# jameshensman/pyvb

Measured on NVIDIA B200. Metric: VB-PCA missing-data rows*iters/sec, higher is better.
Workload: dtype f64

## Files before the change

### pyvb_b200/csrc/kernels_i8.cu

```cuda
#include <cuda.h>
#include <stdio.h>
#include <stdlib.h>

#include "common.cuh"
#include "kernels.h"
#include "ptx.cuh"
#include "umma.cuh"

namespace pyvb {

namespace {

__host__ __device__ constexpr int i_tri(int i) { return i * (i + 1) / 2; }
__host__ __device__ constexpr int i_nc8(int q) { return (i_tri(q) + 31) & ~31; }
constexpr int NPL = 7;
constexpr int BM = 128, BKB = 64, ST = 16, CT = 32;
constexpr int A_B = BM * BKB, B_B = NPL * CT * BKB;
constexpr int NTHR = 10 * 32;

__device__ __forceinline__ double pow2_above(double m) {
    if (!(m > 0.0 && m < 1e300)) return 1.0;
    int e;
    frexp(m, &e);
    return ldexp(1.0, e);
// ... 657 lines not shown
            hi[k] = (unsigned int)(u >> 32);
        }
#pragma unroll
        for (int p = 0; p < NPL; ++p) {
            const unsigned int *w = (p < 4) ? lo : hi;
            const unsigned int sel = (unsigned)(p & 3) | ((unsigned)(4 + (p & 3)) << 4);
            const unsigned int w01 = __byte_perm(w[0], w[1], sel), w23 = __byte_perm(w[2], w[3], sel);
            *reinterpret_cast<unsigned int *>(&sh[(p * CT + lane) * PITCH + r]) = __byte_perm(w01, w23, 0x5410);
        }
    }
    __syncthreads();
    const int nct = gridDim.y;
#pragma unroll
    for (int h = 0; h < 2; ++h) {
        const long long kb = n0 / 64 + h;
        unsigned int *dst = reinterpret_cast<unsigned int *>(ZI + ((size_t)(kb * nct + ct) * (NPL * CT)) * 64);
        for (int w = threadIdx.x; w < NPL * CT * 16; w += 256)
            dst[w] = *reinterpret_cast<const unsigned int *>(&sh[(w >> 4) * PITCH + h * 64 + (w & 15) * 4]);
    }
}

__global__ void __launch_bounds__(256)
prepare_maskT_kernel(long long N, int D, long long npad, const double *__restrict__ X, long long ldx,
                     signed char *__restrict__ maskT) {
    constexpr int PITCH = 132;
    __shared__ __align__(16) signed char sh[32 * PITCH];
    const int d0 = blockIdx.y * 32;
    const long long n0 = (long long)blockIdx.x * 128;
    const int lane = threadIdx.x & 31, warp = threadIdx.x >> 5;
    const int d = d0 + lane;
    for (int r = warp; r < 128; r += 8) {
        const long long n = n0 + r;
        signed char m = 0;
        if (d < D && n < N) {
            const double x = X[n * ldx + d];
            m = (x == x) ? 1 : 0;
        }
        sh[lane * PITCH + r] = m;
    }
    __syncthreads();
#pragma unroll
    for (int h = 0; h < 2; ++h) {
        const long long kb = n0 / 64 + h;
        for (int w = threadIdx.x; w < 32 * 16; w += 256) {
            const int row = w >> 4;
            if (d0 + row < D)
                *reinterpret_cast<unsigned int *>(maskT + ((size_t)kb * D + d0 + row) * 64 + (w & 15) * 4) =
                    *reinterpret_cast<const unsigned int *>(&sh[row * PITCH + h * 64 + (w & 15) * 4]);
        }
    }
}

constexpr int CHK_BLOCKS = 0;
__global__ void __launch_bounds__(128)
stats_i8_check_kernel(int D, int q, const double *__restrict__ ws, int nchunks, const double *__restrict__ cnt,
                      const double *__restrict__ zscale, double *__restrict__ guard, double tol) {
    __shared__ double sh[8];
    const StatLayout L(D, q);
    const int P = i_tri(q), warp = threadIdx.x >> 5, lane = threadIdx.x & 31;
    const int d = blockIdx.x;
    double sz = 0.0;
    for (int c = threadIdx.x; c < P; c += 128) sz = fmax(sz, zscale[c]);
    double dm = 0.0;
    for (int i = warp; i < q; i += 4) {
        const size_t off = L.t1 + (size_t)d * P + i_tri(i) + i;
        double t = 0.0;
        for (int ch = lane; ch < nchunks; ch += 32) t += ws[(size_t)ch * L.len + off];
        dm = fmax(dm, warp_sum(t));
    }
    for (int o = 16; o > 0; o >>= 1) sz = fmax(sz, __shfl_xor_sync(0xffffffffu, sz, o));
    if (lane == 0) {
        sh[warp] = sz;
        sh[4 + warp] = dm;
    }
    __syncthreads();
    if (threadIdx.x == 0) {
        sz = fmax(fmax(sh[0], sh[1]), fmax(sh[2], sh[3])) * 2.7755575615628914e-17;
        dm = fmax(fmax(sh[4], sh[5]), fmax(sh[6], sh[7]));
        if (cnt[d] * sz > tol * dm) atomicAdd(guard + 3, 1.0);
        __threadfence();
        const unsigned int done = atomicAdd(reinterpret_cast<unsigned int *>(guard + 2), 1u);
        if (done == gridDim.x - 1) {
            __threadfence();
            const double t = *reinterpret_cast<volatile double *>(guard + 3);
            guard[0] = t;
            if (t > 0.0) guard[1] += 1.0;
            guard[3] = 0.0;
            *reinterpret_cast<unsigned int *>(guard + 2) = 0u;
        }
    }
}

size_t si8_smem_bytes(int q, int pair = 0) {
    const int ns = pair ? SST_PAIR : SST;
    return 1024 + (size_t)ns * (A_B + (pair ? B_B / 2 : B_B)) + (size_t)((i_tri(q) + q + 31) & ~31) * 8 + (size_t)(2 * ns + 4) * 8 + 16;
}

template <int CL, bool PAIR = false>
__global__ void __launch_bounds__(NTHR, 1)
stats_i8_kernel(const __grid_constant__ CUtensorMap tmA, const __grid_constant__ CUtensorMap tmB, long long N, int D, int q,
                const double *__restrict__ zscale, double *__restrict__ ws, long long rows_per_chunk, int nchunks, int ndb,
                int nct, int ks) {
    extern __shared__ unsigned char smem_dyn[];
    unsigned char *smem = smem_dyn + ((1024u - (smem_u32(smem_dyn) & 1023u)) & 1023u);
    static_assert(!PAIR || CL == 2, "a CTA pair is a cluster of two");
    constexpr int BSZ = PAIR ? B_B / 2 : B_B, STG = A_B + BSZ, NSMAX = PAIR ? SST_PAIR : SST;
    const int NS = NSMAX / ks, SB = ks * STG;
    const int P = i_tri(q), NCZ = (P + q + 31) & ~31;
    unsigned char *st_base = smem;
    double *fcol = reinterpret_cast<double *>(smem + (size_t)NSMAX * STG);
    uint64_t *full = reinterpret_cast<uint64_t *>(fcol + NCZ);
    uint64_t *empty = full + NSMAX;
    uint64_t *tfull = empty + NSMAX;
    uint64_t *tempty = tfull + 2;
    uint32_t *tbase = reinterpret_cast<uint32_t *>(tempty + 2);

    const int tid = threadIdx.x, warp = tid >> 5, lane = tid & 31;
    const int crank = (CL > 1) ? (int)cluster_ctarank() : 0;
    const int ndg = (ndb + CL - 1) / CL;
    const int nitems = ndg * nct * nchunks;
    const int cid = (int)blockIdx.x / CL, ncl = (int)gridDim.x / CL;
    constexpr uint16_t CMASK = (uint16_t)((1u << CL) - 1u);
    for (int c = tid; c < NCZ; c += NTHR) fcol[c] = zscale[c] * 5.5511151231257827e-17;
    if (tid == 0) {
        tma_prefetch_desc(&tmA);
        tma_prefetch_desc(&tmB);
        for (int s = 0; s < NSMAX; ++s) {
            mbar_init(&full[s], 1);
            mbar_init(&empty[s], PAIR ? 1 : CL);
        }
        for (int b = 0; b < 2; ++b) {
            mbar_init(&tfull[b], 1);
            mbar_init(&tempty[b], PAIR ? 16 : 8);
        }
        mbar_fence_init();
    }
    if (warp == 1) {
        if (PAIR) umma::tmem_alloc2(tbase, 512);
        else umma::tmem_alloc(tbase, 512);
    }
    umma::fence_before_sync();
    __syncthreads();
    if (CL > 1) cluster_sync_all();
    umma::fence_after_sync();
    const uint32_t tmem = *tbase;

    auto item_geom = [&](int item, int &chunk, int &db, int &ct, long long &r0, int &nsteps) {
        chunk = item / (ndg * nct);
        const int rem = item - chunk * (ndg * nct);
        const int dg = rem / nct;
        ct = rem - dg * nct;
        db = dg * CL + crank;
        r0 = (long long)chunk * rows_per_chunk;
        long long r1 = r0 + rows_per_chunk;
        if (r1 > N) r1 = N;
        nsteps = (r1 > r0) ? (int)((r1 - r0 + BKB - 1) / BKB) : 0;
    };

    if (warp == 0) {
        const bool leader = elect_one();
        const uint32_t full_l = PAIR ? umma::map_to_cta(full, 0) : 0u;
        int s = 0;
        uint32_t ph = 0;
        for (int item = cid; item < nitems; item += ncl) {
            int chunk, db, ct, nsteps;
            long long r0;
            item_geom(item, chunk, db, ct, r0, nsteps);
            for (int k = 0; k < nsteps; k += ks) {
                const int kc = (nsteps - k < ks) ? nsteps - k : ks;
                umma::mbar_wait_bounded(&empty[s], ph ^ 1);
                if (leader) {
                    if (PAIR) {
                        if (crank == 0) mbar_arrive_expect_tx(&full[s], (uint32_t)(2 * kc * STG));
                    } else {
                        mbar_arrive_expect_tx(&full[s], (uint32_t)(kc * (A_B + B_B)));
                    }
                    for (int h = 0; h < kc; ++h) {
                        unsigned char *st = st_base + (size_t)s * SB + (size_t)h * STG;
                        const long long kb = r0 / BKB + k + h;
                        if (PAIR) {
                            tma_load_3d_i8_pair(st, &tmA, 0, (int)(kb * D + db * BM), 0, full_l + (uint32_t)s * 8u);
                            tma_load_3d_i8_pair(st + A_B, &tmB, 0, (int)((kb * nct + ct) * (NPL * CT) + crank * (NPL * CT / 2)), 0,
                                                full_l + (uint32_t)s * 8u);
                        } else {
                            tma_load_3d_i8(st, &tmA, 0, (int)(kb * D + db * BM), 0, &full[s]);
                            if (CL == 1)
                                tma_load_3d_i8(st + A_B, &tmB, 0, (int)((kb * nct + ct) * (NPL * CT)), 0, &full[s]);
                            else
                                tma_load_3d_i8_mc(st + A_B + crank * (B_B / CL), &tmB, 0,
                                                  (int)((kb * nct + ct) * (NPL * CT) + crank * (NPL * CT / CL)), 0, &full[s], CMASK);
                        }
                    }
                }
                __syncwarp();
                if (++s == NS) {
                    s = 0;
                    ph ^= 1;
                }
            }
        }
    } else if (warp == 1) {
        const bool leader = elect_one() && (!PAIR || crank == 0);
        const uint32_t idesc = umma::idesc_s8_s32(PAIR ? 2 * BM : BM, NPL * CT);
        const uint64_t adesc0 = umma::desc_kmajor_sw64(smem_u32(st_base), 0), bdesc0 = umma::desc_kmajor_sw64(smem_u32(st_base + A_B), 0);
        int s = 0, tl = 0;
        uint32_t ph = 0;
        for (int item = (PAIR && crank != 0) ? nitems : cid; item < nitems; item += ncl, ++tl) {
            int chunk, db, ct, nsteps;
            long long r0;
            item_geom(item, chunk, db, ct, r0, nsteps);
            const int buf = tl & 1;
            umma::mbar_wait_bounded(&tempty[buf], (uint32_t)(((tl >> 1) & 1) ^ 1));
            umma::fence_after_sync();
            const uint32_t dacc = tmem + (uint32_t)(buf * 256);
            for (int k = 0; k < nsteps; k += ks) {
                const int kc = (nsteps - k < ks) ? nsteps - k : ks;
                umma::mbar_wait_bounded(&full[s], ph);
                umma::fence_after_sync();
                if (leader) {
                    for (int h = 0; h < kc; ++h) {
                        const uint64_t off = (uint64_t)((s * SB + h * STG) >> 4);
                        if (PAIR) {
                            umma::mma_i8_pair(dacc, adesc0 + off, bdesc0 + off, idesc, (k + h) ? 1u : 0u);
                            umma::mma_i8_pair(dacc, adesc0 + off + 2, bdesc0 + off + 2, idesc, 1u);
                        } else {
                            umma::mma_i8(dacc, adesc0 + off, bdesc0 + off, idesc, (k + h) ? 1u : 0u);
                            umma::mma_i8(dacc, adesc0 + off + 2, bdesc0 + off + 2, idesc, 1u);
                        }
                    }
                    if (PAIR) umma::mma_commit_pair(&empty[s]);
                    else if (CL == 1) umma::mma_commit(&empty[s]);
                    else mma_commit_mc(&empty[s], CMASK);
                }
                __syncwarp();
                if (++s == NS) {
                    s = 0;
                    ph ^= 1;
                }
            }
            if (leader) {
                if (PAIR) umma::mma_commit_pair(&tfull[buf]);
                else umma::mma_commit(&tfull[buf]);
            }
            __syncwarp();
        }
    } else {
        const StatLayout L(D, q);
        const int wq = warp & 3, half = (warp - 2) >> 2;
        const uint32_t tempty_l = PAIR ? umma::map_to_cta(tempty, 0) : 0u;
        int tl = 0;
        for (int item = cid; item < nitems; item += ncl, ++tl) {
            int chunk, db, ct, nsteps;
            long long r0;
            item_geom(item, chunk, db, ct, r0, nsteps);
            const int buf = tl & 1;
            const int d = db * BM + wq * 32 + lane;
            const int c0 = ct * CT + half * 16;
            double *out = ws + (size_t)chunk * L.len;
            umma::mbar_wait_bounded(&tfull[buf], (uint32_t)((tl >> 1) & 1));
            umma::fence_after_sync();
            const uint32_t taddr = tmem + (uint32_t)(buf * 256 + half * 16) + ((uint32_t)(wq * 32) << 16);
#pragma unroll
            for (int ch = 0; ch < 2; ++ch) {
                uint32_t a[NPL][8];
                if (nsteps > 0) {
#pragma unroll
                    for (int p = 0; p < NPL; ++p) tmem_ld8(taddr + (uint32_t)(p * CT + ch * 8), a[p]);
                    umma::tmem_ld_wait();
                }
#pragma unroll
                for (int k = 0; k < 8; ++k) {
                    double v = 0.0;
                    if (nsteps > 0) {
#pragma unroll
                        for (int p = NPL - 1; p >= 0; --p) v = fma(v, 256.0, i2d((int)a[p][k]));
                    }
                    const int c = c0 + ch * 8 + k;
                    if (d < D) {
                        if (c < P) out[L.t1 + (size_t)d * P + c] = fcol[c] * v;
                        else if (c < P + q) out[L.bst + (size_t)d * q + (c - P)] = fcol[c] * v;
                    }
                }
            }
            umma::fence_before_sync();
            __syncwarp();
            if (lane == 0) {
                if (PAIR) umma::mbar_arrive_cluster(tempty_l + (uint32_t)buf * 8u);
                else mbar_arrive(&tempty[buf]);
            }
        }
    }
    umma::fence_before_sync();
    __syncthreads();
    if (CL > 1) cluster_sync_all();
    if (warp == 1) {
        if (PAIR) umma::tmem_dealloc2(tmem, 512);
        else umma::tmem_dealloc(tmem, 512);
    }
}

constexpr int SF_CONV = 8;
constexpr int SF_NTHR = (2 + 8 + SF_CONV) * 32;
constexpr int SF_STG = 2 * A_B + B_B;
constexpr int SF_NSMAX = 8;

int sf_stages(int q) {
    const size_t fixed = 1024 + (size_t)stats_i8_ncols(q) * 8 + (size_t)(2 * SF_NSMAX + 2) * 8 + 16;
    const int ns = (int)((227 * 1024 - fixed) / SF_STG);
    return ns < SF_NSMAX ? ns : SF_NSMAX;
}
size_t sf_smem_bytes(int q, int ns) {
    return 1024 + (size_t)ns * SF_STG + (size_t)stats_i8_ncols(q) * 8 + (size_t)(2 * ns + 2) * 8 + 16;
}

__global__ void __launch_bounds__(SF_NTHR, 1)
stats_i8_fused_kernel(const __grid_constant__ CUtensorMap tmA, long long N, int D, int q, const double *__restrict__ MZ, int ldmz,
                      const double *__restrict__ zscale, double *__restrict__ ws, long long rows_per_chunk, int nchunks,
                      int ndb, int nct, int ns) {
    extern __shared__ unsigned char smem_dyn[];
    unsigned char *smem = smem_dyn + ((1024u - (smem_u32(smem_dyn) & 1023u)) & 1023u);
    const int P = i_tri(q), NCZ = nct * CT;
    unsigned char *st_base = smem;
    double *fcol = reinterpret_cast<double *>(smem + (size_t)ns * SF_STG);
    uint64_t *full = reinterpret_cast<uint64_t *>(fcol + NCZ);
    uint64_t *empty = full + ns;
    uint64_t *tfull = empty + ns;
    uint64_t *tempty = tfull + 1;
    uint32_t *tbase = reinterpret_cast<uint32_t *>(tempty + 1);

    const int tid = threadIdx.x, warp = tid >> 5, lane = tid & 31;
    const int nitems = nct * nchunks;
    for (int c = tid; c < NCZ; c += SF_NTHR) fcol[c] = zscale[c] * 5.5511151231257827e-17;
    if (tid == 0) {
        tma_prefetch_desc(&tmA);
        for (int s = 0; s < ns; ++s) {
            mbar_init(&full[s], 1 + SF_CONV / 2);
            mbar_init(&empty[s], 1);
        }
        mbar_init(tfull, 1);
        mbar_init(tempty, 8);
        mbar_fence_init();
    }
    if (warp == 1) umma::tmem_alloc(tbase, 512);
    umma::fence_before_sync();
    __syncthreads();
    umma::fence_after_sync();
    const uint32_t tmem = *tbase;

    auto item_geom = [&](int item, int &chunk, int &ct, long long &r0, int &nsteps) {
        chunk = item / nct;
        ct = item - chunk * nct;
        r0 = (long long)chunk * rows_per_chunk;
        long long r1 = r0 + rows_per_chunk;
        if (r1 > N) r1 = N;
        nsteps = (r1 > r0) ? (int)((r1 - r0 + BKB - 1) / BKB) : 0;
    };

    if (warp == 0) {
        const bool leader = elect_one();
        int s = 0;
        uint32_t ph = 0;
        for (int item = blockIdx.x; item < nitems; item += gridDim.x) {
            int chunk, ct, nsteps;
            long long r0;
            item_geom(item, chunk, ct, r0, nsteps);
            for (int k = 0; k < nsteps; ++k) {
                umma::mbar_wait_bounded(&empty[s], ph ^ 1);
                if (leader) {
                    mbar_arrive_expect_tx(&full[s], (uint32_t)(ndb * A_B));
                    const long long kb = r0 / BKB + k;
                    for (int b = 0; b < ndb; ++b)
                        tma_load_3d_i8(st_base + (size_t)s * SF_STG + b * A_B, &tmA, 0, (int)(kb * D + b * BM), 0, &full[s]);
                }
                __syncwarp();
                if (++s == ns) {
                    s = 0;
                    ph ^= 1;
                }
            }
        }
    } else if (warp == 1) {
        const bool leader = elect_one();
        const uint32_t idesc = umma::idesc_s8_s32(BM, NPL * CT);
        const uint64_t adesc0 = umma::desc_kmajor_sw64(smem_u32(st_base), 0);
        const uint64_t bdesc0 = umma::desc_kmajor_sw64(smem_u32(st_base + 2 * A_B), 0);
        int s = 0, tl = 0;
        uint32_t ph = 0;
        for (int item = blockIdx.x; item < nitems; item += gridDim.x, ++tl) {
            int chunk, ct, nsteps;
            long long r0;
            item_geom(item, chunk, ct, r0, nsteps);
            umma::mbar_wait_bounded(tempty, (uint32_t)((tl & 1) ^ 1));
            umma::fence_after_sync();
            for (int k = 0; k < nsteps; ++k) {
                umma::mbar_wait_bounded(&full[s], ph);
                umma::fence_after_sync();
                if (leader) {
                    const uint64_t off = (uint64_t)((s * SF_STG) >> 4);
                    for (int b = 0; b < ndb; ++b) {
                        const uint32_t dacc = tmem + (uint32_t)(b * 256);
                        const uint64_t ad = adesc0 + off + (uint64_t)(b * (A_B >> 4));
                        umma::mma_i8(dacc, ad, bdesc0 + off, idesc, k ? 1u : 0u);
                        umma::mma_i8(dacc, ad + 2, bdesc0 + off + 2, idesc, 1u);
                    }
                    umma::mma_commit(&empty[s]);
                }
                __syncwarp();
                if (++s == ns) {
                    s = 0;
                    ph ^= 1;
                }
            }
            if (leader) umma::mma_commit(tfull);
            __syncwarp();
        }
    } else if (warp < 10) {
        const StatLayout L(D, q);
        const int wq = warp & 3, half = (warp - 2) >> 2;
        int tl = 0;
        for (int item = blockIdx.x; item < nitems; item += gridDim.x, ++tl) {
            int chunk, ct, nsteps;
            long long r0;
            item_geom(item, chunk, ct, r0, nsteps);
            const int c0 = ct * CT + half * 16;
            double *out = ws + (size_t)chunk * L.len;
            umma::mbar_wait_bounded(tfull, (uint32_t)(tl & 1));
            umma::fence_after_sync();
            for (int b = 0; b < ndb; ++b) {
                const int d = b * BM + wq * 32 + lane;
                const uint32_t taddr = tmem + (uint32_t)(b * 256 + half * 16) + ((uint32_t)(wq * 32) << 16);
#pragma unroll
                for (int ch = 0; ch < 2; ++ch) {
                    uint32_t a[NPL][8];
                    if (nsteps > 0) {
#pragma unroll
                        for (int p = 0; p < NPL; ++p) tmem_ld8(taddr + (uint32_t)(p * CT + ch * 8), a[p]);
                        umma::tmem_ld_wait();
                    }
#pragma unroll
                    for (int k = 0; k < 8; ++k) {
                        double v = 0.0;
                        if (nsteps > 0) {
#pragma unroll
                            for (int p = NPL - 1; p >= 0; --p) v = fma(v, 256.0, i2d((int)a[p][k]));
                        }
                        const int c = c0 + ch * 8 + k;
                        if (d < D) {
                            if (c < P) out[L.t1 + (size_t)d * P + c] = fcol[c] * v;
                            else if (c < P + q) out[L.bst + (size_t)d * q + (c - P)] = fcol[c] * v;
                        }
                    }
                }
            }
            umma::fence_before_sync();
            __syncwarp();
            if (lane == 0) mbar_arrive(tempty);
        }
    } else {
        const int cw = warp - 10, grp = cw >> 2, rq = cw & 3, rot = lane >> 3;
        const int nvalid = P + q;
        constexpr unsigned long long BIAS = 0x0080808080808080ULL;
        const uint32_t wbase = (uint32_t)(lane * 64 + ((rq ^ ((lane >> 1) & 3)) << 4));
        struct Pos {
            int item, k, nsteps, ct;
            long long r0;
        };
        auto settle = [&](Pos &p) {
            while (p.item < nitems && p.k >= p.nsteps) {
                p.k -= p.nsteps;
                p.item += gridDim.x;
                int chunk;
                if (p.item < nitems) item_geom(p.item, chunk, p.ct, p.r0, p.nsteps);
            }
        };
        auto load = [&](const Pos &p, double (&x)[16]) {
            const int c = p.ct * CT + lane;
            const bool cv = p.item < nitems && c < nvalid;
            const long long nb = p.r0 + (long long)p.k * BKB + rq * 16;
#pragma unroll
            for (int g = 0; g < 4; ++g)
#pragma unroll
                for (int kk = 0; kk < 4; ++kk) {
                    const long long n = nb + 4 * ((g + rot) & 3) + kk;
                    x[g * 4 + kk] = (cv && n < N) ? __ldcs(MZ + n * ldmz + c) : 0.0;
                }
        };
        Pos cur;
        cur.item = blockIdx.x;
        cur.k = grp;
        cur.nsteps = 0;
        {
            int chunk;
            if (cur.item < nitems) item_geom(cur.item, chunk, cur.ct, cur.r0, cur.nsteps);
        }
        settle(cur);
        double xv[16], xn[16];
        load(cur, xv);
        for (int j = grp; cur.item < nitems; j += 2) {
            Pos nxt = cur;
            nxt.k += 2;
            settle(nxt);
            load(nxt, xn);
            const int s = j % ns;
            umma::mbar_wait_bounded(&empty[s], (uint32_t)(((j / ns) & 1) ^ 1));
            const int c = cur.ct * CT + lane;
            const double inv = c < nvalid ? 18014398509481984.0 / zscale[c] : 0.0;
            unsigned char *bt = st_base + (size_t)s * SF_STG + 2 * A_B;
#pragma unroll
            for (int g = 0; g < 4; ++g) {
                const int qd = (g + rot) & 3;
                unsigned int lo[4], hi[4];
#pragma unroll
                for (int kk = 0; kk < 4; ++kk) {
                    double t = xv[g * 4 + kk] * inv;
                    t = (fabs(t) <= 18014398509481984.0) ? t : 0.0;
                    const unsigned long long u = ((unsigned long long)__double2ll_rn(t) + BIAS) ^ BIAS;
                    lo[kk] = (unsigned int)u;
                    hi[kk] = (unsigned int)(u >> 32);
                }
#pragma unroll
                for (int p = 0; p < NPL; ++p) {
                    const unsigned int *w = (p < 4) ? lo : hi;
                    const unsigned int sel = (unsigned)(p & 3) | ((unsigned)(4 + (p & 3)) << 4);
                    const unsigned int w01 = __byte_perm(w[0], w[1], sel), w23 = __byte_perm(w[2], w[3], sel);
                    *reinterpret_cast<unsigned int *>(bt + p * (CT * BKB) + wbase + qd * 4) = __byte_perm(w01, w23, 0x5410);
                }
            }
            fence_async_smem();
            __syncwarp();
            if (lane == 0) mbar_arrive(&full[s]);
            cur = nxt;
#pragma unroll
            for (int i = 0; i < 16; ++i) xv[i] = xn[i];
        }
    }
    umma::fence_before_sync();
    __syncthreads();
    if (warp == 1) umma::tmem_dealloc(tmem, 512);
}


__global__ void __launch_bounds__(128, 1) bench_umma_kernel(int iters, int n, int kind, int mode, const unsigned char *src,
                                                           long long *clk_out) {
    extern __shared__ unsigned char smem_dyn[];
    unsigned char *smem = smem_dyn + ((1024u - (smem_u32(smem_dyn) & 1023u)) & 1023u);
    constexpr int STG = A_B + 256 * BKB;
    __shared__ uint64_t bar, cbar[4], lbar[2];
    __shared__ uint32_t tb;
    __shared__ int stop;
    for (int i = threadIdx.x; i < 4 * STG / 4; i += 128) reinterpret_cast<uint32_t *>(smem)[i] = 0x01010101u;
    if (threadIdx.x == 0) {
        mbar_init(&bar, 1);
        for (int i = 0; i < 4; ++i) mbar_init(&cbar[i], 1);
        mbar_init(&lbar[0], 1);
        mbar_init(&lbar[1], 1);
        stop = 0;
        mbar_fence_init();
    }
    if (threadIdx.x < 32) umma::tmem_alloc(&tb, 512);
    fence_async_smem();
    umma::fence_before_sync();
    __syncthreads();
    umma::fence_after_sync();
    const uint32_t tmem = tb;
    if (threadIdx.x == 0) {
        const uint32_t idesc = kind == 0 ? umma::idesc_s8_s32(BM, n) : umma::idesc_bf16_f32(BM, n, 0, 0);
        const long long t0 = clock64();
        for (int it = 0; it < iters; ++it) {
            const uint32_t d = tmem + (uint32_t)((it & 1) * 256);
            const uint32_t a0 = smem_u32(smem) + ((mode & 1) ? (uint32_t)((it & 3) * STG) : 0u), b0 = a0 + A_B;
            if (kind == 0) {
                umma::mma_i8(d, umma::desc_kmajor_sw64(a0, 0), umma::desc_kmajor_sw64(b0, 0), idesc, 1u);
                umma::mma_i8(d, umma::desc_kmajor_sw64(a0, 1), umma::desc_kmajor_sw64(b0, 1), idesc, 1u);
            } else {
                umma::mma_bf16(d, umma::desc_kmajor_sw64(a0, 0), umma::desc_kmajor_sw64(b0, 0), idesc, 1u);
                umma::mma_bf16(d, umma::desc_kmajor_sw64(a0, 1), umma::desc_kmajor_sw64(b0, 1), idesc, 1u);
            }
            if (mode & 2) umma::mma_commit(&cbar[it & 3]);
        }
        umma::mma_commit(&bar);
        umma::mbar_wait_bounded(&bar, 0);
        clk_out[blockIdx.x] = clock64() - t0;
        *reinterpret_cast<volatile int *>(&stop) = 1;
    } else if (threadIdx.x == 32 && (mode & 4)) {
        unsigned char *dst = smem + 4 * STG;
        uint32_t ph[2] = {0, 0};
        int k = 0;
        const unsigned char *g = src + (size_t)blockIdx.x * (1 << 20);
        mbar_arrive_expect_tx(&lbar[0], B_B);
        bulk_g2s(dst, g, B_B, &lbar[0]);
        mbar_arrive_expect_tx(&lbar[1], B_B);
        bulk_g2s(dst + B_B, g + B_B, B_B, &lbar[1]);
        while (!*reinterpret_cast<volatile int *>(&stop)) {
            const int b = k & 1;
            umma::mbar_wait_bounded(&lbar[b], ph[b]);
            ph[b] ^= 1;
            ++k;
            mbar_arrive_expect_tx(&lbar[b], B_B);
            bulk_g2s(dst + b * B_B, g + (size_t)((k * B_B) & ((1 << 20) - 32768)), B_B, &lbar[b]);
        }
        umma::mbar_wait_bounded(&lbar[0], ph[0]);
        umma::mbar_wait_bounded(&lbar[1], ph[1]);
        clk_out[148 + blockIdx.x] = k;
    }
    umma::fence_before_sync();
    __syncthreads();
    if (threadIdx.x < 32) umma::tmem_dealloc(tmem, 512);
}

}

cudaError_t launch_bench_umma(int blocks, int iters, int n, int kind, int mode, const void *src, long long *clk_out,
                              cudaStream_t st) {
    const size_t smem = 1024 + 4 * (A_B + 256 * BKB) + 2 * B_B;
    cudaError_t e = cudaFuncSetAttribute(bench_umma_kernel, cudaFuncAttributeMaxDynamicSharedMemorySize, (int)smem);
    if (e != cudaSuccess) return e;
    bench_umma_kernel<<<blocks, 128, smem, st>>>(iters, n, kind, mode, static_cast<const unsigned char *>(src), clk_out);
    return cudaGetLastError();
}

bool i8_supported(int D, int q) {
    return (q == 16 || q == 32 || q == 64) && D >= 64 && (D % 64) == 0 && i8_stages(D, q, 1) >= 2;
}
size_t i8_digits_bytes(int D, int q) { return (size_t)(i_nc8(q) / CT) * NPL * CT * D; }
size_t i8_mask_bytes(long long N, int D) { return (size_t)((N + BM - 1) / BM * BM) * (size_t)D; }
int i8_ncols(int q) { return i_nc8(q); }

cudaError_t launch_prepare_mask_i8(long long N, int D, const double *X, long long ldx, void *mask, cudaStream_t st) {
    if (N <= 0) return cudaSuccess;
    long long b = (((N + BM - 1) / BM * BM) * (long long)(D / 4) + 255) / 256;
    if (b > 148 * 16) b = 148 * 16;
    prepare_mask_i8_kernel<<<(unsigned)b, 256, 0, st>>>(N, D, X, ldx, static_cast<signed char *>(mask));
    return cudaGetLastError();
}

cudaError_t launch_pack_g_i8(int D, int q, const double *Gw, int ldg, void *GI, double *gscale, double *gl, cudaStream_t st) {
    pack_g_i8_kernel<<<i_nc8(q), 256, 0, st>>>(D, q, Gw, ldg, static_cast<signed char *>(GI), gscale, gl);
    return cudaGetLastError();
}

cudaError_t launch_zstep_i8(long long N, int D, int q, const void *mask, const void *GI, const double *P0,
                            const double *gscale, const double *gl, double *MZ, int ldmz, cudaStream_t st) {
    if (N <= 0) return cudaSuccess;
    if (!i8_supported(D, q)) return cudaErrorNotSupported;
    const I8Geom g(q);
    const long long nrb = (N + BM - 1) / BM;
    int cl = i8_cluster_size();
    while (cl > 1 && nrb < 2LL * cl) cl >>= 1;
    CUtensorMap tmA, tmB;
    const uint64_t nk = (uint64_t)(D / BKB);
    if ((uint64_t)nrb * nk * BM >= (1ULL << 31)) return cudaErrorNotSupported;
    cudaError_t e = make_map_u8_3d(&tmA, mask, BKB, (uint64_t)nrb * nk * BM, 1, BKB, BM);
    if (e != cudaSuccess) return e;
    e = make_map_u8_3d(&tmB, GI, BKB, nk * g.NCT * (NPL * CT), 1, BKB, NPL * CT / cl);
    if (e != cudaSuccess) return e;
    CUtensorMap tmO;
    {
        EncodeTiledFn enc = get_encode_i8();
        if (!enc) return cudaErrorNotSupported;
        cuuint64_t dims[2] = {(cuuint64_t)g.PP, (cuuint64_t)N};
        cuuint64_t strides[1] = {(cuuint64_t)ldmz * sizeof(double)};
        cuuint32_t box[2] = {16, 32}, es[2] = {1, 1};
        CUresult r = enc(&tmO, CU_TENSOR_MAP_DATA_TYPE_FLOAT64, 2, MZ, dims, strides, box, es, CU_TENSOR_MAP_INTERLEAVE_NONE,
                         CU_TENSOR_MAP_SWIZZLE_128B, CU_TENSOR_MAP_L2_PROMOTION_L2_128B, CU_TENSOR_MAP_FLOAT_OOB_FILL_NONE);
        if (r != CUDA_SUCCESS) return cudaErrorInvalidValue;
    }
    const int pair = (cl == 2 && i8_pair_mode() && i8_stages(D, q, i8_hstage(D, q), 0) < 8) ? 1 : 0;
    const int hstage = pair ? ((i8_stages(D, q, 0, 1) < 12 && i8_stages(D, q, 1, 1) > i8_stages(D, q, 0, 1)) ? 1 : 0) : i8_hstage(D, q);
    static int adbl_on = -1;
    if (adbl_on < 0) {
        const char *ev = getenv("PYVB_I8_ADBL");
        adbl_on = (ev && ev[0] == '0') ? 0 : 1;
    }
    const int adbl = (adbl_on && !pair && i8_stages(D, q, hstage, 0, 1) >= ST / 2) ? 1 : 0;
    int nst = i8_stages(D, q, hstage, pair, adbl);
    if (nst < 2) return cudaErrorNotSupported;
    const size_t smem = i8_smem_bytes(D, q, nst, hstage, pair, adbl);
    static int ks_env = -1;
    if (ks_env < 0) {
        const char *ev = getenv("PYVB_I8_KS");
        ks_env = ev ? atoi(ev) : 0;
    }
    int ks = (ks_env == 1 || ks_env == 2) ? ks_env : 2;
    if ((nk % 2) != 0 || nst < 4) ks = 1;
    if (ks == 2) nst /= 2;
    CUtensorMap tmO8;
    {
        EncodeTiledFn enc = get_encode_i8();
        cuuint64_t dims[2] = {(cuuint64_t)g.PP, (cuuint64_t)N};
        cuuint64_t strides[1] = {(cuuint64_t)ldmz * sizeof(double)};
        cuuint32_t box[2] = {8, 32}, es[2] = {1, 1};
        CUresult r = enc(&tmO8, CU_TENSOR_MAP_DATA_TYPE_FLOAT64, 2, MZ, dims, strides, box, es, CU_TENSOR_MAP_INTERLEAVE_NONE,
                         CU_TENSOR_MAP_SWIZZLE_64B, CU_TENSOR_MAP_L2_PROMOTION_L2_128B, CU_TENSOR_MAP_FLOAT_OOB_FILL_NONE);
        if (r != CUDA_SUCCESS) return cudaErrorInvalidValue;
    }
    long long gl_ = (nrb + cl - 1) / cl * cl;
    const int grid = (int)(gl_ < 148 ? gl_ : 148 / cl * cl);
    auto kern = cl == 4 ? zstep_i8_kernel<4> : cl == 2 ? (pair ? zstep_i8_kernel<2, true> : zstep_i8_kernel<2>) : zstep_i8_kernel<1>;
    e = cudaFuncSetAttribute(kern, cudaFuncAttributeMaxDynamicSharedMemorySize, (int)smem);
    if (e != cudaSuccess) return e;
    static long long *prof = nullptr;
    static int prof_on = -1;
    if (prof_on < 0) {
        prof_on = getenv("PYVB_I8_PROF") ? 1 : 0;
        if (prof_on && cudaMalloc(&prof, 148 * 10 * sizeof(long long)) != cudaSuccess) prof_on = 0;
    }
    e = launch_cluster(kern, grid, NTHR, smem, cl, st, tmA, tmB, tmO, tmO8, N, D, q, P0, gscale, gl, (int)nrb, nst, hstage, adbl,
                       prof_on ? prof : (long long *)nullptr, ks);
    if (prof_on && e == cudaSuccess) {
        long long h[148 * 10];
        cudaStreamSynchronize(st);
        cudaMemcpy(h, prof, sizeof(h), cudaMemcpyDeviceToHost);
        double a[10] = {0};
        for (int b = 0; b < grid; ++b)
            for (int k = 0; k < 10; ++k) a[k] += (double)h[b * 10 + k] / grid;
        fprintf(stderr, "[i8 prof] N=%lld D=%d q=%d cl=%d nst=%d total %.0f clk | producer: empty %.0f aempty %.0f | mma: full %.0f tempty %.0f afull %.0f | epilogue(w2): tfull %.0f store-read %.0f\n",
                N, D, q, cl, nst, a[9], a[0], a[1], a[3], a[4], a[5], a[6], a[7]);
    }
    return e;
}

bool stats_i8_supported(int D, int q) { return (q == 16 || q == 32 || q == 64) && D >= 16 && (D % 16) == 0; }
int stats_i8_ncols(int q) { return (i_tri(q) + q + 31) & ~31; }
long long stats_i8_npad(long long N) { return (N + 127) / 128 * 128; }
size_t stats_i8_digits_bytes(long long N, int q) { return (size_t)stats_i8_ncols(q) * NPL * (size_t)stats_i8_npad(N); }
size_t stats_i8_maskt_bytes(long long N, int D) { return (size_t)D * (size_t)stats_i8_npad(N) + (size_t)BM * BKB; }
size_t stats_i8_scratch_len(int q, int ldmz) { return (size_t)CM_BLOCKS * 2 * ldmz + stats_i8_ncols(q) + 8 + CHK_BLOCKS; }
double *stats_i8_guard(double *scratch, int q, int ldmz) { return scratch + (size_t)CM_BLOCKS * 2 * ldmz + stats_i8_ncols(q); }

cudaError_t launch_stats_i8_check(int D, int q, const double *ws, int nchunks, const double *xcache, double *scratch,
                                  int ldmz, double tol, cudaStream_t st) {
    stats_i8_check_kernel<<<D, 128, 0, st>>>(D, q, ws, nchunks, xcache, scratch + (size_t)CM_BLOCKS * 2 * ldmz,
                                                  stats_i8_guard(scratch, q, ldmz), tol);
    return cudaGetLastError();
}

static int stats_pair_min_d() {
    static int d = -1;
    if (d < 0) {
        const char *e = getenv("PYVB_I8_STATS_PAIR_D");
        d = e ? atoi(e) : 512;
    }
    return d;
}
static long long gcd_ll(long long a, long long b) { return b ? gcd_ll(b, a % b) : a; }
int stats_i8_nchunks(long long N, int D, int q) {
    const int cl = i8_cluster_size();
    const long long ncl = 148 / cl;
    const long long per = (long long)(((D + BM - 1) / BM + cl - 1) / cl) * (stats_i8_ncols(q) / CT);
    const long long step = ncl / gcd_ll(ncl, per);
    long long by_rows = N / (32LL * BKB);
    if (by_rows < 1) by_rows = 1;
    long long k = (6 * ncl + per * step - 1) / (per * step);
    if (k < 1) k = 1;
    long long c = k * step;
    if (c > by_rows) c = (by_rows >= step) ? (by_rows / step) * step : by_rows;
    const long long cmin = (N + (1LL << 23) - 1) >> 23;
    if (c < cmin) c = cmin;
    if (c > 1024) c = 1024;
    return (int)c;
}
long long stats_i8_rows_per_chunk(long long N, int nchunks) {
    long long rpc = (N + nchunks - 1) / nchunks;
    rpc = (rpc + BKB - 1) / BKB * BKB;
    return rpc < BKB ? BKB : rpc;
}

cudaError_t launch_prepare_maskT_i8(long long N, int D, const double *X, long long ldx, void *maskT, cudaStream_t st) {
    if (N <= 0) return cudaSuccess;
    dim3 grid((unsigned)((N + 127) / 128), (unsigned)((D + 31) / 32));
    prepare_maskT_kernel<<<grid, 256, 0, st>>>(N, D, stats_i8_npad(N), X, ldx, static_cast<signed char *>(maskT));
    return cudaGetLastError();
}

bool stats_i8_fused(int D) {
    const char *e = getenv("PYVB_I8_FUSED");
    return (D + BM - 1) / BM <= 2 && !(e && e[0] == '0');
}

cudaError_t launch_stats_i8(long long N, int D, int q, const void *maskT, const double *MZ, int ldmz, void *ZI,
                            double *scratch, double *ws, int nchunks, const double *zsums, int nzblk, int zkw, int trusted,
                            const double *logdet, const double **zs_out, int *nzblk_out, int *zkw_out, cudaStream_t st) {
    if (N <= 0) return cudaSuccess;
    const int P = i_tri(q), NCZ = stats_i8_ncols(q), nct = NCZ / CT, ndb = (D + BM - 1) / BM;
    const long long npad = stats_i8_npad(N);
    const int orow = gw_woff(q) + q;
    double *pm = scratch, *zscale = scratch + (size_t)CM_BLOCKS * 2 * ldmz;
    if (!(zsums != nullptr && nzblk > 0 && trusted)) {
        if (logdet == nullptr) return cudaErrorInvalidValue;
        int nblk = CM_BLOCKS;
        long long rpb = (N + nblk - 1) / nblk;
        if (rpb < 64) rpb = 64;
        nblk = (int)((N + rpb - 1) / rpb);
        mzpart_kernel<<<nblk, 256, (size_t)(2 * ldmz + 4) * sizeof(double), st>>>(N, ldmz, orow, MZ, logdet, pm, rpb);
        zsums = pm;
        nzblk = nblk;
        zkw = 2 * orow + 4;
    }
    *zs_out = zsums;
    *nzblk_out = nzblk;
    *zkw_out = zkw;
    colmax_reduce_kernel<<<(NCZ + 7) / 8, 256, 0, st>>>(NCZ, P + q, zkw, zsums + orow + 4, nzblk, zscale);
    cudaError_t e = cudaGetLastError();
    if (e != cudaSuccess) return e;
    const cuuint64_t nkb = (cuuint64_t)(npad / BKB);
    EncodeTiledFn enc = get_encode_i8();
    if (!enc) return cudaErrorNotSupported;
    if (nkb * (cuuint64_t)D + BM >= (1ULL << 31) || nkb * nct * (NPL * CT) >= (1ULL << 31)) return cudaErrorNotSupported;
    const cuuint32_t es[3] = {1, 1, 1};
    CUtensorMap tmA;
    {
        cuuint64_t da[3] = {BKB, nkb * D + BM, 1}, sa[2] = {BKB, (nkb * D + BM) * BKB};
        cuuint32_t ba[3] = {BKB, BM, 1};
        CUresult r = enc(&tmA, CU_TENSOR_MAP_DATA_TYPE_UINT8, 3, const_cast<void *>(maskT), da, sa, ba, es,
                         CU_TENSOR_MAP_INTERLEAVE_NONE, CU_TENSOR_MAP_SWIZZLE_64B, CU_TENSOR_MAP_L2_PROMOTION_L2_128B,
                         CU_TENSOR_MAP_FLOAT_OOB_FILL_NONE);
        if (r != CUDA_SUCCESS) return cudaErrorInvalidValue;
    }
    const long long rpc = stats_i8_rows_per_chunk(N, nchunks);
    if (stats_i8_fused(D)) {
        const int ns = sf_stages(q);
        const size_t smem = sf_smem_bytes(q, ns);
        e = cudaFuncSetAttribute(stats_i8_fused_kernel, cudaFuncAttributeMaxDynamicSharedMemorySize, (int)smem);
        if (e != cudaSuccess) return e;
        const long long nitems = (long long)nct * nchunks;
        const int grid = (int)(nitems < 148 ? nitems : 148);
        stats_i8_fused_kernel<<<grid, SF_NTHR, smem, st>>>(tmA, N, D, q, MZ, ldmz, (const double *)zscale, ws, rpc, nchunks, ndb,
                                                           nct, ns);
        return cudaGetLastError();
    }
    if (ZI == nullptr) return cudaErrorInvalidValue;
    dim3 gd((unsigned)((N + 127) / 128), (unsigned)nct);
    digitize_kernel<<<gd, 256, 0, st>>>(N, npad, ldmz, P + q, MZ, zscale, static_cast<signed char *>(ZI));
    e = cudaGetLastError();
    if (e != cudaSuccess) return e;
    CUtensorMap tmB;
    {
        cuuint64_t db[3] = {BKB, nkb * nct * (NPL * CT), 1}, sb[2] = {BKB, nkb * nct * (NPL * CT) * BKB};
        cuuint32_t bb[3] = {BKB, (cuuint32_t)(NPL * CT / i8_cluster_size()), 1};
        CUresult r = enc(&tmB, CU_TENSOR_MAP_DATA_TYPE_UINT8, 3, ZI, db, sb, bb, es, CU_TENSOR_MAP_INTERLEAVE_NONE,
                         CU_TENSOR_MAP_SWIZZLE_64B, CU_TENSOR_MAP_L2_PROMOTION_L2_128B, CU_TENSOR_MAP_FLOAT_OOB_FILL_NONE);
        if (r != CUDA_SUCCESS) return cudaErrorInvalidValue;
    }
    const int cl = i8_cluster_size();
    const int pair = (cl == 2 && i8_pair_mode() && ndb >= 2 && D >= stats_pair_min_d()) ? 1 : 0;
    const size_t smem = si8_smem_bytes(q, pair);
    auto kern = cl == 4 ? stats_i8_kernel<4> : cl == 2 ? (pair ? stats_i8_kernel<2, true> : stats_i8_kernel<2>) : stats_i8_kernel<1>;
    e = cudaFuncSetAttribute(kern, cudaFuncAttributeMaxDynamicSharedMemorySize, (int)smem);
    if (e != cudaSuccess) return e;
    const long long nitems = (long long)((ndb + cl - 1) / cl) * nct * nchunks;
    const int grid = (int)(nitems < 148 / cl ? nitems : 148 / cl) * cl;
    static int ks_env = -1;
    if (ks_env < 0) {
        const char *ev = getenv("PYVB_I8_STATS_KS");
        ks_env = ev ? atoi(ev) : 0;
    }
    const int ks = (ks_env >= 1 && ks_env <= 4) ? ks_env : 2;
    return launch_cluster(kern, grid, NTHR, smem, cl, st, tmA, tmB, N, D, q, (const double *)zscale, ws, rpc, nchunks, ndb,
                          nct, ks);
}

}
```

Measured before the change: 410.9 million.

## Stream MZ tiles into converter warps via TMA ring instead of per-lane loads

Converter warps previously read MZ rows with per-lane streaming global loads, software double-buffered in registers. Each converter warp now has a small shared-memory ring of TMA 2D tiles carrying an L2 evict-first hint, prefetched a few steps ahead and guarded by per-slot mbarriers. The per-column reciprocal of zscale is cached across iterations, and the shared memory spent on the ring can reduce the number of pipeline stages. Optional clock64 wait profiling, enabled by an environment variable, is also added.

Result: faster. 440.9 million (median of 6 runs) (+7.3%).

```diff
diff --git a/pyvb_b200/csrc/kernels_i8.cu b/pyvb_b200/csrc/kernels_i8.cu
--- a/pyvb_b200/csrc/kernels_i8.cu
+++ b/pyvb_b200/csrc/kernels_i8.cu
@@ -983,43 +983,72 @@
 constexpr int SF_CONV = 8;
 constexpr int SF_NTHR = (2 + 8 + SF_CONV) * 32;
 constexpr int SF_STG = 2 * A_B + B_B;
+constexpr int SF_ZB = 16 * CT * 8;
 constexpr int SF_NSMAX = 8;
-
+constexpr int SF_PROF = 24;
+
+size_t sf_smem_bytes(int q, int ns, int nz) {
+    return 1024 + (size_t)ns * SF_STG + (size_t)SF_CONV * nz * SF_ZB + (size_t)stats_i8_ncols(q) * 8 +
+           (size_t)(2 * ns + 2 + SF_CONV * nz) * 8 + 16;
+}
+constexpr int SF_NZ = 2;
 int sf_stages(int q) {
-    const size_t fixed = 1024 + (size_t)stats_i8_ncols(q) * 8 + (size_t)(2 * SF_NSMAX + 2) * 8 + 16;
-    const int ns = (int)((227 * 1024 - fixed) / SF_STG);
-    return ns < SF_NSMAX ? ns : SF_NSMAX;
-}
-size_t sf_smem_bytes(int q, int ns) {
-    return 1024 + (size_t)ns * SF_STG + (size_t)stats_i8_ncols(q) * 8 + (size_t)(2 * ns + 2) * 8 + 16;
+    int ns = SF_NSMAX;
+    while (ns > 2 && sf_smem_bytes(q, ns, SF_NZ) > 227 * 1024) --ns;
+    return ns;
+}
+
+__device__ __forceinline__ void tma_load_2d_hint(const void *dst_smem, const void *tmap, int c0, int c1, uint64_t *bar,
+                                                 uint64_t policy) {
+    asm volatile(
+        "cp.async.bulk.tensor.2d.shared::cluster.global.mbarrier::complete_tx::bytes.L2::cache_hint [%0], [%1, {%2, %3}], [%4], "
+        "%5;" ::"r"(smem_u32(dst_smem)),
+        "l"(tmap), "r"(c0), "r"(c1), "r"(smem_u32(bar)), "l"(policy)
+        : "memory");
 }
 
 __global__ void __launch_bounds__(SF_NTHR, 1)
-stats_i8_fused_kernel(const __grid_constant__ CUtensorMap tmA, long long N, int D, int q, const double *__restrict__ MZ, int ldmz,
+stats_i8_fused_kernel(const __grid_constant__ CUtensorMap tmA, const __grid_constant__ CUtensorMap tmZ, long long N, int D, int q,
                       const double *__restrict__ zscale, double *__restrict__ ws, long long rows_per_chunk, int nchunks,
-                      int ndb, int nct, int ns) {
+                      int ndb, int nct, int ns, int nz, long long *prof) {
+    long long w0 = 0, w1 = 0;
+    const long long tstart = clock64();
+#define PROF_WAIT(acc, stmt)                    \
+    do {                                        \
+        if (prof) {                             \
+            const long long t_ = clock64();     \
+            stmt;                               \
+            acc += clock64() - t_;              \
+        } else {                                \
+            stmt;                               \
+        }                                       \
+    } while (0)
     extern __shared__ unsigned char smem_dyn[];
     unsigned char *smem = smem_dyn + ((1024u - (smem_u32(smem_dyn) & 1023u)) & 1023u);
     const int P = i_tri(q), NCZ = nct * CT;
     unsigned char *st_base = smem;
-    double *fcol = reinterpret_cast<double *>(smem + (size_t)ns * SF_STG);
+    unsigned char *zbuf = smem + (size_t)ns * SF_STG;
+    double *fcol = reinterpret_cast<double *>(zbuf + (size_t)SF_CONV * nz * SF_ZB);
     uint64_t *full = reinterpret_cast<uint64_t *>(fcol + NCZ);
     uint64_t *empty = full + ns;
     uint64_t *tfull = empty + ns;
     uint64_t *tempty = tfull + 1;
-    uint32_t *tbase = reinterpret_cast<uint32_t *>(tempty + 1);
+    uint64_t *zfull = tempty + 1;
+    uint32_t *tbase = reinterpret_cast<uint32_t *>(zfull + SF_CONV * nz);
 
     const int tid = threadIdx.x, warp = tid >> 5, lane = tid & 31;
     const int nitems = nct * nchunks;
     for (int c = tid; c < NCZ; c += SF_NTHR) fcol[c] = zscale[c] * 5.5511151231257827e-17;
     if (tid == 0) {
         tma_prefetch_desc(&tmA);
+        tma_prefetch_desc(&tmZ);
         for (int s = 0; s < ns; ++s) {
             mbar_init(&full[s], 1 + SF_CONV / 2);
             mbar_init(&empty[s], 1);
         }
         mbar_init(tfull, 1);
         mbar_init(tempty, 8);
+        for (int i = 0; i < SF_CONV * nz; ++i) mbar_init(&zfull[i], 1);
         mbar_fence_init();
     }
     if (warp == 1) umma::tmem_alloc(tbase, 512);
@@ -1046,7 +1075,7 @@
             long long r0;
             item_geom(item, chunk, ct, r0, nsteps);
             for (int k = 0; k < nsteps; ++k) {
-                umma::mbar_wait_bounded(&empty[s], ph ^ 1);
+                PROF_WAIT(w0, umma::mbar_wait_bounded(&empty[s], ph ^ 1));
                 if (leader) {
                     mbar_arrive_expect_tx(&full[s], (uint32_t)(ndb * A_B));
                     const long long kb = r0 / BKB + k;
@@ -1071,10 +1100,10 @@
             int chunk, ct, nsteps;
             long long r0;
             item_geom(item, chunk, ct, r0, nsteps);
-            umma::mbar_wait_bounded(tempty, (uint32_t)((tl & 1) ^ 1));
+            PROF_WAIT(w1, umma::mbar_wait_bounded(tempty, (uint32_t)((tl & 1) ^ 1)));
             umma::fence_after_sync();
             for (int k = 0; k < nsteps; ++k) {
-                umma::mbar_wait_bounded(&full[s], ph);
+                PROF_WAIT(w0, umma::mbar_wait_bounded(&full[s], ph));
                 umma::fence_after_sync();
                 if (leader) {
                     const uint64_t off = (uint64_t)((s * SF_STG) >> 4);
@@ -1105,7 +1134,7 @@
             item_geom(item, chunk, ct, r0, nsteps);
             const int c0 = ct * CT + half * 16;
             double *out = ws + (size_t)chunk * L.len;
-            umma::mbar_wait_bounded(tfull, (uint32_t)(tl & 1));
+            PROF_WAIT(w0, umma::mbar_wait_bounded(tfull, (uint32_t)(tl & 1)));
             umma::fence_after_sync();
             for (int b = 0; b < ndb; ++b) {
                 const int d = b * BM + wq * 32 + lane;
@@ -1142,6 +1171,11 @@
         const int nvalid = P + q;
         constexpr unsigned long long BIAS = 0x0080808080808080ULL;
         const uint32_t wbase = (uint32_t)(lane * 64 + ((rq ^ ((lane >> 1) & 3)) << 4));
+        const double *zring = reinterpret_cast<const double *>(zbuf + (size_t)cw * nz * SF_ZB);
+        uint64_t *zb = zfull + cw * nz;
+        const bool zlead = elect_one();
+        uint64_t policy = 0;
+        if (zlead) asm volatile("createpolicy.fractional.L2::evict_first.b64 %0, 1.0;" : "=l"(policy));
         struct Pos {
             int item, k, nsteps, ct;
             long long r0;
@@ -1154,17 +1188,10 @@
                 if (p.item < nitems) item_geom(p.item, chunk, p.ct, p.r0, p.nsteps);
             }
         };
-        auto load = [&](const Pos &p, double (&x)[16]) {
-            const int c = p.ct * CT + lane;
-            const bool cv = p.item < nitems && c < nvalid;
-            const long long nb = p.r0 + (long long)p.k * BKB + rq * 16;
-#pragma unroll
-            for (int g = 0; g < 4; ++g)
-#pragma unroll
-                for (int kk = 0; kk < 4; ++kk) {
-                    const long long n = nb + 4 * ((g + rot) & 3) + kk;
-                    x[g * 4 + kk] = (cv && n < N) ? __ldcs(MZ + n * ldmz + c) : 0.0;
-                }
+        auto issue = [&](const Pos &p, int slot) {
+            mbar_arrive_expect_tx(&zb[slot], (uint32_t)SF_ZB);
+            tma_load_2d_hint(zring + slot * (SF_ZB / 8), &tmZ, p.ct * CT, (int)(p.r0 + (long long)p.k * BKB + rq * 16), &zb[slot],
+                             policy);
         };
         Pos cur;
         cur.item = blockIdx.x;
@@ -1175,17 +1202,37 @@
             if (cur.item < nitems) item_geom(cur.item, chunk, cur.ct, cur.r0, cur.nsteps);
         }
         settle(cur);
-        double xv[16], xn[16];
-        load(cur, xv);
-        for (int j = grp; cur.item < nitems; j += 2) {
-            Pos nxt = cur;
-            nxt.k += 2;
-            settle(nxt);
-            load(nxt, xn);
+        Pos ahead = cur;
+        for (int i = 0; i < nz && ahead.item < nitems; ++i) {
+            if (zlead) issue(ahead, i);
+            ahead.k += 2;
+            settle(ahead);
+        }
+        int ict = -1;
+        double inv = 0.0;
+        for (int j = grp, zt = 0; cur.item < nitems; j += 2, ++zt) {
+            const int zs = zt % nz;
+            PROF_WAIT(w0, umma::mbar_wait_bounded(&zb[zs], (uint32_t)((zt / nz) & 1)));
+            double xv[16];
+            const double *zr = zring + zs * (SF_ZB / 8) + lane;
+#pragma unroll
+            for (int g = 0; g < 4; ++g)
+#pragma unroll
+                for (int kk = 0; kk < 4; ++kk) xv[g * 4 + kk] = zr[(4 * ((g + rot) & 3) + kk) * CT];
+            __syncwarp();
+            fence_async_smem();
+            if (ahead.item < nitems) {
+                if (zlead) issue(ahead, zs);
+                ahead.k += 2;
+                settle(ahead);
+            }
+            if (cur.ct != ict) {
+                ict = cur.ct;
+                const int c = ict * CT + lane;
+                inv = c < nvalid ? 18014398509481984.0 / zscale[c] : 0.0;
+            }
             const int s = j % ns;
-            umma::mbar_wait_bounded(&empty[s], (uint32_t)(((j / ns) & 1) ^ 1));
-            const int c = cur.ct * CT + lane;
-            const double inv = c < nvalid ? 18014398509481984.0 / zscale[c] : 0.0;
+            PROF_WAIT(w1, umma::mbar_wait_bounded(&empty[s], (uint32_t)(((j / ns) & 1) ^ 1)));
             unsigned char *bt = st_base + (size_t)s * SF_STG + 2 * A_B;
 #pragma unroll
             for (int g = 0; g < 4; ++g) {
@@ -1210,10 +1257,23 @@
             fence_async_smem();
             __syncwarp();
             if (lane == 0) mbar_arrive(&full[s]);
-            cur = nxt;
-#pragma unroll
-            for (int i = 0; i < 16; ++i) xv[i] = xn[i];
-        }
+            cur.k += 2;
+            settle(cur);
+        }
+    }
+#undef PROF_WAIT
+    if (prof && lane == 0 && (warp < 3 || warp >= 10)) {
+        long long *o = prof + (size_t)blockIdx.x * SF_PROF;
+        if (warp < 2) {
+            o[warp] = w0;
+            if (warp == 1) o[2] = w1;
+        } else if (warp == 2) {
+            o[3] = w0;
+        } else {
+            o[4 + (warp - 10)] = w0;
+            o[12 + (warp - 10)] = w1;
+        }
+        if (warp == 0) o[20] = clock64() - tstart;
     }
     umma::fence_before_sync();
     __syncthreads();
@@ -1500,15 +1560,46 @@
     }
     const long long rpc = stats_i8_rows_per_chunk(N, nchunks);
     if (stats_i8_fused(D)) {
-        const int ns = sf_stages(q);
-        const size_t smem = sf_smem_bytes(q, ns);
+        CUtensorMap tmZ;
+        {
+            cuuint64_t dz[2] = {(cuuint64_t)(P + q), (cuuint64_t)N}, sz[1] = {(cuuint64_t)ldmz * sizeof(double)};
+            cuuint32_t bz[2] = {CT, 16};
+            CUresult r = enc(&tmZ, CU_TENSOR_MAP_DATA_TYPE_FLOAT64, 2, const_cast<double *>(MZ), dz, sz, bz, es,
+                             CU_TENSOR_MAP_INTERLEAVE_NONE, CU_TENSOR_MAP_SWIZZLE_NONE, CU_TENSOR_MAP_L2_PROMOTION_NONE,
+                             CU_TENSOR_MAP_FLOAT_OOB_FILL_NONE);
+            if (r != CUDA_SUCCESS) return cudaErrorInvalidValue;
+        }
+        const int ns = sf_stages(q), nz = SF_NZ;
+        const size_t smem = sf_smem_bytes(q, ns, nz);
         e = cudaFuncSetAttribute(stats_i8_fused_kernel, cudaFuncAttributeMaxDynamicSharedMemorySize, (int)smem);
         if (e != cudaSuccess) return e;
         const long long nitems = (long long)nct * nchunks;
         const int grid = (int)(nitems < 148 ? nitems : 148);
-        stats_i8_fused_kernel<<<grid, SF_NTHR, smem, st>>>(tmA, N, D, q, MZ, ldmz, (const double *)zscale, ws, rpc, nchunks, ndb,
-                                                           nct, ns);
-        return cudaGetLastError();
+        static long long *prof = nullptr;
+        static int prof_on = -1;
+        if (prof_on < 0) {
+            prof_on = getenv("PYVB_I8_PROF") ? 1 : 0;
+            if (prof_on && cudaMalloc(&prof, 148 * SF_PROF * sizeof(long long)) != cudaSuccess) prof_on = 0;
+        }
+        stats_i8_fused_kernel<<<grid, SF_NTHR, smem, st>>>(tmA, tmZ, N, D, q, (const double *)zscale, ws, rpc, nchunks, ndb, nct,
+                                                           ns, nz, prof_on ? prof : (long long *)nullptr);
+        e = cudaGetLastError();
+        if (prof_on && e == cudaSuccess) {
+            long long h[148 * SF_PROF];
+            cudaStreamSynchronize(st);
+            cudaMemcpy(h, prof, sizeof(h), cudaMemcpyDeviceToHost);
+            double a[SF_PROF] = {0};
+            for (int b = 0; b < grid; ++b)
+                for (int k = 0; k < SF_PROF; ++k) a[k] += (double)h[b * SF_PROF + k] / grid;
+            double cl = 0, ce = 0;
+            for (int w = 0; w < SF_CONV; ++w) {
+                cl += a[4 + w] / SF_CONV;
+                ce += a[12 + w] / SF_CONV;
+            }
+            fprintf(stderr, "[i8 stats prof] N=%lld D=%d q=%d ns=%d nz=%d total %.0f clk | producer: empty %.0f | mma: full %.0f tempty %.0f | epilogue(w2): tfull %.0f | converters: loads %.0f empty %.0f\n",
+                    N, D, q, ns, nz, a[20], a[0], a[1], a[2], a[3], cl, ce);
+        }
+        return e;
     }
     if (ZI == nullptr) return cudaErrorInvalidValue;
     dim3 gd((unsigned)((N + 127) / 128), (unsigned)nct);
```
